# AhmedHumais/E-RAFT

Measured on AMD Instinct MI355X. Metric: CorrBlock build+lookup frame-pairs/sec & HBM GB/s at DSEC 480×640, 1–8 GPUs, higher is better.
Workload: dtype f32; 1 GPU; CorrBlock build + 12 lookups, dsec fmaps [1,256,60,80], 4 levels, radius 4; global_batch=1, launch=hipgraph, parallelism=replicas x1 (independent frame pairs per GPU)

## Files before the change

### e-raft_amd/csrc/corr_build_bf16.hip

```cpp
#include <algorithm>
#include <atomic>
#include <cmath>

#include "corr_build_common.h"

namespace corr {

typedef __bf16 bfx8_t __attribute__((ext_vector_type(8)));
typedef unsigned u32x4_t __attribute__((ext_vector_type(4)));
typedef float f32x4_t __attribute__((ext_vector_type(4)));

namespace bf16b {

constexpr int kStepK = 32;
constexpr int kPieces = 3;
constexpr int kRecU = kPieces * 64;
constexpr int kPatchRows = 8;
constexpr int kWaves = 4, kQPerWave = 32;
constexpr int kQPerWG = kWaves * kQPerWave;
constexpr int kRing = 3;
constexpr int kSlotBytes = kPatchRows * kPieces * 1024;
constexpr int kLds = kRing * kSlotBytes;
constexpr int kDmaPerWave = kPatchRows * kPieces / kWaves;
constexpr int kQLoads = 2 * kPieces;
constexpr int kPixBytes = kStepK * kPieces * 2;

struct Geom {
    int S, NQp, NQB, NQG, Hp, CB, Wp;
};

inline Geom geom(int D, int NQ, int H, int W) {
    Geom g;
    g.S = (D + kStepK - 1) / kStepK;
    g.NQp = (NQ + kQPerWG - 1) / kQPerWG * kQPerWG;
    g.NQB = g.NQp / 16;
    g.NQG = g.NQp / kQPerWG;
    g.Hp = (H + kPatchRows - 1) / kPatchRows * kPatchRows;
    g.CB = (W + 15) / 16;
    g.Wp = g.CB * 16;
    return g;
}

struct PackArgs {
    const float *f[2];
    u32x4_t *pk[2];
    int np[2];
    int nblk[2];
    int img[2];
    int D, S, W, CB, y0, y1, z0;
};

template <int R = 1>
__global__ __launch_bounds__(256) void bf16_pack_kernel(PackArgs a) {
    const int z = blockIdx.z + a.z0, b = blockIdx.y;
    const int nblk = a.nblk[z];
    const int lane = threadIdx.x & 63, ci = lane & 15, grp = lane >> 4;
    const int NP = a.np[z];
    float v[R][8];
    bool live[R];
    size_t dst[R];
#pragma unroll
    for (int r = 0; r < R; ++r) {
        const int rec = (blockIdx.x * R + r) * 4 + (threadIdx.x >> 6);
        live[r] = rec < a.S * nblk;
        const int s = live[r] ? rec / nblk : 0, blk = live[r] ? rec - s * nblk : 0;
        int n, iblk;
        bool valid;
        if (z == 0) {
            n = blk * 16 + ci;
            valid = n < a.np[0];
            iblk = blk;
        } else {
            const int TCp = 4 * a.CB, ty = blk / TCp, tx = blk - ty * TCp;
            const int ly = 4 * ty + (ci >> 2), x = 4 * tx + (ci & 3);
            valid = a.y0 + ly < a.y1 && x < a.W;
            n = ly * a.W + x;
            iblk = (a.y0 >> 2) * TCp + blk;
        }
        valid = valid && live[r];
        const int k0 = s * kStepK + 8 * grp;
        const float *src = a.f[z] + (size_t)b * a.D * NP + (valid ? n : 0);
#pragma unroll
        for (int j = 0; j < 8; ++j) v[r][j] = (valid && k0 + j < a.D) ? src[(size_t)(k0 + j) * NP] : 0.f;
        dst[r] = (((size_t)b * a.S + s) * a.img[z] + iblk) * kRecU + lane;
    }
#pragma unroll
    for (int r = 0; r < R; ++r) {
        if (!live[r]) continue;
        unsigned hh[4], mm[4], ll[4];
#pragma unroll
        for (int j = 0; j < 4; ++j) split3(v[r][2 * j], v[r][2 * j + 1], hh[j], mm[j], ll[j]);
        const u32x4_t h{hh[0], hh[1], hh[2], hh[3]}, m{mm[0], mm[1], mm[2], mm[3]}, l{ll[0], ll[1], ll[2], ll[3]};
        u32x4_t *out = a.pk[z] + dst[r];
        out[0] = h;
        out[64] = m;
        out[128] = l;
    }
}

struct Args {
    const u32x4_t *pq, *pt;
    float *lvl[kFusedLevels];
    int B, H, W, N, NQ, S, nlev;
    int NQp, NQB, NQG, Hp, CB, npatch;
    int py0;
    int exact;
    float inv_s, s;
    int order;
    int gq;
    int nqh, npq;
};

__device__ __forceinline__ Tile xcd_block_tile(const Args &p, int t) {
    Tile o;
    const int per_b = p.npatch * p.NQG;
    o.b = t / per_b;
    int r = t - o.b * per_b;
    int q0 = 0, q1 = 0, p0 = 0, p1 = 0;
    for (int i = 0; i < p.nqh; ++i) {
        const int qa = i * p.NQG / p.nqh, qb = (i + 1) * p.NQG / p.nqh;
        const int rows = (qb - qa) * p.npatch;
        if (r < rows) {
            for (int j = 0; j < p.npq; ++j) {
                const int pa = j * p.npatch / p.npq, pb = (j + 1) * p.npatch / p.npq;
                const int sz = (qb - qa) * (pb - pa);
                if (r < sz) {
                    q0 = qa, q1 = qb, p0 = pa, p1 = pb;
                    break;
                }
                r -= sz;
            }
            break;
        }
        r -= rows;
    }
    (void)q1;
    const int np = p1 - p0;
    o.qg = q0 + r / np;
    const int patch = p0 + r % np;
    o.py = patch / p.CB;
    o.cb = patch - o.py * p.CB;
    return o;
}

template <int SS, int NR, bool ACC2, int VF = 0, bool FAST = false>
__device__ __forceinline__ void build_tile(const Args &p, const Tile tl) {
    constexpr int QS = ACC2 ? 3 : 4, QD = QS - 1;
    constexpr int WV = kWaves, QPWG = kQPerWG, DPW = kDmaPerWave;
    extern __shared__ __attribute__((aligned(16))) char smem_bf16[];
    char *smem = smem_bf16;

    const int b = tl.b, y0 = tl.py * kPatchRows, x0 = tl.cb * 16;
    const int tid = threadIdx.x, lane = tid & 63;
    const int w = __builtin_amdgcn_readfirstlane(tid >> 6);
    const int ci = lane & 15, grp = lane >> 4;
    const int qb0 = tl.qg * (QPWG / 16) + 2 * w;
    const int S = SS > 0 ? SS : p.S;
    const bool qact = qb0 * 16 < p.NQ;

    const int TCp = 4 * p.CB;
    const size_t tstep = (size_t)p.Hp * p.CB * kRecU;
    const u32x4_t *tbase = p.pt + (((size_t)b * S * (p.Hp >> 2) + (y0 >> 2)) * TCp + 4 * tl.cb) * kRecU + lane;
    unsigned toff[DPW];
#pragma unroll
    for (int m = 0; m < DPW; ++m) {
        const int pc = w + WV * m, rp = pc / kPieces;
        toff[m] = (unsigned)(((rp >> 2) * TCp + (rp & 3)) * kRecU + (pc % kPieces) * 64);
    }
    const size_t qstep = (size_t)p.NQB * kRecU;
    const uint32_t lds_base = (uint32_t)(uintptr_t)(lds_void_t *)smem;
    const u32x4_t *qsrc = p.pq + ((size_t)b * S * p.NQB + qb0) * kRecU + lane;

    u32x4_t qv[QS][2][kPieces];
    auto issue_q = [&](int s, int slot) __attribute__((always_inline)) {
#pragma unroll
        for (int i = 0; i < 2; ++i)
#pragma unroll
            for (int c = 0; c < kPieces; ++c) {
                if constexpr (VF & 1)
                    asm volatile("global_load_dwordx4 %0, %1, off" : "=v"(qv[slot][i][c]) : "v"(qsrc + s * qstep + i * kRecU + c * 64) : "memory");
                else
                    qv[slot][i][c] = qsrc[s * qstep + i * kRecU + c * 64];
            }
    };
    auto issue_t = [&](int s, int slot) __attribute__((always_inline)) {
        const uint32_t base = lds_base + slot * kSlotBytes;
        const u32x4_t *src = tbase + s * tstep;
#pragma unroll
        for (int m = 0; m < DPW; ++m) dma16(src + toff[m], base + (w + WV * m) * 1024);
    };

    f32x4_t acc[2][kPatchRows], acs[2][kPatchRows];
#pragma unroll
    for (int i = 0; i < 2; ++i)
#pragma unroll
        for (int r = 0; r < kPatchRows; ++r) acc[i][r] = acs[i][r] = f32x4_t{0.f, 0.f, 0.f, 0.f};

    auto compute = [&](int tslot, int qslot) __attribute__((always_inline)) {
        const u32x4_t *A = reinterpret_cast<const u32x4_t *>(smem + tslot * kSlotBytes);
        bfx8_t qh[2], qm[2], ql[2];
#pragma unroll
        for (int i = 0; i < 2; ++i) {
            qh[i] = __builtin_bit_cast(bfx8_t, qv[qslot][i][0]);
            qm[i] = __builtin_bit_cast(bfx8_t, qv[qslot][i][1]);
            ql[i] = __builtin_bit_cast(bfx8_t, qv[qslot][i][2]);
        }
        bfx8_t th[2], tm[2], tl8[2];
        th[0] = __builtin_bit_cast(bfx8_t, A[lane]);
        tm[0] = __builtin_bit_cast(bfx8_t, A[64 + lane]);
        tl8[0] = __builtin_bit_cast(bfx8_t, A[128 + lane]);
        if constexpr (ACC2) {
#pragma unroll
            for (int r = 0; r < NR; ++r) {
                const int c = r & 1;
                if (r + 1 < NR) {
                    th[c ^ 1] = __builtin_bit_cast(bfx8_t, A[(3 * r + 3) * 64 + lane]);
                    tm[c ^ 1] = __builtin_bit_cast(bfx8_t, A[(3 * r + 4) * 64 + lane]);
                    tl8[c ^ 1] = __builtin_bit_cast(bfx8_t, A[(3 * r + 5) * 64 + lane]);
                }
#pragma unroll
                for (int i = 0; i < 2; ++i) acs[i][r] = __builtin_amdgcn_mfma_f32_16x16x32_bf16(tl8[c], qh[i], acs[i][r], 0, 0, 0);
#pragma unroll
                for (int i = 0; i < 2; ++i) acs[i][r] = __builtin_amdgcn_mfma_f32_16x16x32_bf16(th[c], ql[i], acs[i][r], 0, 0, 0);
#pragma unroll
                for (int i = 0; i < 2; ++i) acs[i][r] = __builtin_amdgcn_mfma_f32_16x16x32_bf16(tm[c], qm[i], acs[i][r], 0, 0, 0);
#pragma unroll
                for (int i = 0; i < 2; ++i) acs[i][r] = __builtin_amdgcn_mfma_f32_16x16x32_bf16(tm[c], qh[i], acs[i][r], 0, 0, 0);
#pragma unroll
                for (int i = 0; i < 2; ++i) acs[i][r] = __builtin_amdgcn_mfma_f32_16x16x32_bf16(th[c], qm[i], acs[i][r], 0, 0, 0);
#pragma unroll
                for (int i = 0; i < 2; ++i) acc[i][r] = __builtin_amdgcn_mfma_f32_16x16x32_bf16(th[c], qh[i], acc[i][r], 0, 0, 0);
            }
            __builtin_amdgcn_sched_group_barrier(0x100, 3, 0);
#pragma unroll
            for (int r = 0; r < NR; ++r) {
                if (r + 1 < NR) __builtin_amdgcn_sched_group_barrier(0x100, 3, 0);
                __builtin_amdgcn_sched_group_barrier(0x008, 12, 0);
            }
        } else {
            f32x4_t t[2][2];
#pragma unroll
            for (int r = 0; r < NR; ++r) {
                const int c = r & 1;
                if (r + 1 < NR) {
                    th[c ^ 1] = __builtin_bit_cast(bfx8_t, A[(3 * r + 3) * 64 + lane]);
                    tm[c ^ 1] = __builtin_bit_cast(bfx8_t, A[(3 * r + 4) * 64 + lane]);
                    tl8[c ^ 1] = __builtin_bit_cast(bfx8_t, A[(3 * r + 5) * 64 + lane]);
                }
                const f32x4_t z = {0.f, 0.f, 0.f, 0.f};
#pragma unroll
                for (int i = 0; i < 2; ++i) t[c][i] = __builtin_amdgcn_mfma_f32_16x16x32_bf16(tl8[c], qh[i], z, 0, 0, 0);
#pragma unroll
                for (int i = 0; i < 2; ++i) t[c][i] = __builtin_amdgcn_mfma_f32_16x16x32_bf16(th[c], ql[i], t[c][i], 0, 0, 0);
#pragma unroll
                for (int i = 0; i < 2; ++i) t[c][i] = __builtin_amdgcn_mfma_f32_16x16x32_bf16(tm[c], qm[i], t[c][i], 0, 0, 0);
#pragma unroll
                for (int i = 0; i < 2; ++i) t[c][i] = __builtin_amdgcn_mfma_f32_16x16x32_bf16(tm[c], qh[i], t[c][i], 0, 0, 0);
#pragma unroll
                for (int i = 0; i < 2; ++i) t[c][i] = __builtin_amdgcn_mfma_f32_16x16x32_bf16(th[c], qm[i], t[c][i], 0, 0, 0);
#pragma unroll
                for (int i = 0; i < 2; ++i) t[c][i] = __builtin_amdgcn_mfma_f32_16x16x32_bf16(th[c], qh[i], t[c][i], 0, 0, 0);
                if (r > 0) {
#pragma unroll
                    for (int i = 0; i < 2; ++i) acc[i][r - 1] += t[c ^ 1][i];
                }
            }
#pragma unroll
            for (int i = 0; i < 2; ++i) acc[i][NR - 1] += t[(NR - 1) & 1][i];
            __builtin_amdgcn_sched_group_barrier(0x100, 3, 0);
#pragma unroll
            for (int r = 0; r < NR; ++r) {
                if (r + 1 < NR) __builtin_amdgcn_sched_group_barrier(0x100, 3, 0);
                __builtin_amdgcn_sched_group_barrier(0x008, 12, 0);
                if (r > 0) __builtin_amdgcn_sched_group_barrier(0x002, 8, 0);
            }
            __builtin_amdgcn_sched_group_barrier(0x002, 8, 0);
        }
    };

    if constexpr (SS > 0) {
        if constexpr ((VF & 2) != 0) __builtin_amdgcn_s_setprio(1);
        issue_q(0, 0);
        if (SS > 1) issue_q(1, 1);
        issue_t(0, 0);
        if (QD > 2 && SS > 2) issue_q(2, 2);
        if (SS > 1) issue_t(1, 1);
#pragma unroll
        for (int s = 0; s < SS; ++s) {
            const int younger = s == 0 ? (QD > 2 && SS > 2 ? kQLoads : 0) + (SS > 1 ? DPW : 0)
                                       : (s - 1 + QD < SS ? kQLoads : 0) + (s + 1 < SS ? DPW : 0);
            if (younger == kQLoads + DPW) wait_vmcnt_barrier<kQLoads + DPW>();
            else if (younger == DPW) wait_vmcnt_barrier<DPW>();
            else if (younger == kQLoads) wait_vmcnt_barrier<kQLoads>();
            else wait_vmcnt_barrier<0>();
            const int qs = s % QS;
#pragma unroll
            for (int i = 0; i < 2; ++i)
                asm volatile("" : "+v"(qv[qs][i][0]), "+v"(qv[qs][i][1]), "+v"(qv[qs][i][2]));
            if (s + QD < SS) issue_q(s + QD, (s + QD) % QS);
            if (s + 2 < SS) issue_t(s + 2, (s + 2) % kRing);
            if (qact) compute(s % kRing, qs);
        }
        if constexpr ((VF & 2) != 0) __builtin_amdgcn_s_setprio(0);
    } else {
        asm volatile("s_waitcnt vmcnt(0)" ::: "memory");
        for (int s = 0; s < S; ++s) {
            issue_q(s, 0);
            issue_t(s, 0);
            wait_vmcnt_barrier<0>();
            if (qact) compute(0, 0);
            asm volatile("s_waitcnt lgkmcnt(0)\n\ts_barrier" ::: "memory");
        }
    }

    const int H = p.H, W = p.W, NQ = p.NQ, nlev = FAST ? 4 : p.nlev;
    const int H1 = H >> 1, W1 = W >> 1, H2 = H >> 2, W2 = W >> 2, H3 = H >> 3, W3 = W >> 3;
    const int TC0 = map_tcols(W), TC1 = map_tcols(W1), TC2 = map_tcols(W2), TC3 = map_tcols(W3);
    const int R0 = 4 * map_tiles(H), R1 = 4 * map_tiles(H1), R2 = 4 * map_tiles(H2), R3 = 4 * map_tiles(H3);
    const size_t M0 = map_floats(H, W), M1 = map_floats(H1, W1), M2 = map_floats(H2, W2), M3 = map_floats(H3, W3);
    const int h = grp >> 1, k = grp & 1;
    float l2s[2][2];
#pragma unroll
    for (int i = 0; i < 2; ++i) {
        const int q = (qb0 + i) * 16 + ci;
        const bool qok = q < NQ;
        const size_t qrow = (size_t)b * NQ + q;
        float v[kPatchRows][4];
#pragma unroll
        for (int r = 0; r < kPatchRows; ++r)
#pragma unroll
            for (int g = 0; g < 4; ++g) v[r][g] = (ACC2 ? split_sum(acc[i][r][g], acs[i][r][g]) : acc[i][r][g]) * p.inv_s;
        if (qok && nlev > 0) {
            float *m0 = p.lvl[0] + qrow * M0;
#pragma unroll
            for (int rp = 0; rp < kPatchRows; ++rp) {
                const int Y = y0 + 4 * (rp >> 2) + grp, T = (x0 >> 2) + (rp & 3);
                if (Y < R0 && 4 * T < W)
                    *reinterpret_cast<float4 *>(m0 + map_row4(Y, T, TC0)) = make_float4(v[rp][0], v[rp][1], v[rp][2], v[rp][3]);
            }
        }
        float l1[2][4];
#pragma unroll
        for (int tr = 0; tr < 2; ++tr) {
            float top[2][4], bot[2][4];
#pragma unroll
            for (int j = 0; j < 2; ++j)
#pragma unroll
                for (int c = 0; c < 4; ++c) {
                    const float mine = k ? v[4 * tr + 2 + j][c] : v[4 * tr + j][c];
                    const float give = k ? v[4 * tr + j][c] : v[4 * tr + 2 + j][c];
                    const float got = __shfl_xor(give, 16);
                    top[j][c] = k ? got : mine;
                    bot[j][c] = k ? mine : got;
                }
#pragma unroll
            for (int m = 0; m < 4; ++m) {
                const int j = m >> 1, c = 2 * (m & 1);
                l1[tr][m] = pool4(top[j][c], top[j][c + 1], bot[j][c], bot[j][c + 1]);
            }
            const int Y1 = (y0 >> 1) + 2 * tr + h, T1 = (x0 >> 3) + k;
            if (qok && nlev > 1 && Y1 < R1 && 4 * T1 < W1)
                *reinterpret_cast<float4 *>(p.lvl[1] + qrow * M1 + map_row4(Y1, T1, TC1)) =
                    make_float4(l1[tr][0], l1[tr][1], l1[tr][2], l1[tr][3]);
        }
        float top[4], bot[4];
#pragma unroll
        for (int m = 0; m < 4; ++m) {
            const float give = h ? l1[0][m] : l1[1][m];
            const float got = __shfl_xor(give, 32);
            top[m] = h ? got : l1[0][m];
            bot[m] = h ? l1[1][m] : got;
        }
#pragma unroll
        for (int j = 0; j < 2; ++j) l2s[i][j] = pool4(top[2 * j], top[2 * j + 1], bot[2 * j], bot[2 * j + 1]);
    }
    {
        const float g0 = __shfl_xor(k ? l2s[0][0] : l2s[1][0], 16), g1 = __shfl_xor(k ? l2s[0][1] : l2s[1][1], 16);
        const float o0 = k ? l2s[1][0] : l2s[0][0], o1 = k ? l2s[1][1] : l2s[0][1];
        const float4 o = k ? make_float4(g0, g1, o0, o1) : make_float4(o0, o1, g0, g1);
        const int q = (qb0 + k) * 16 + ci, Y2 = (y0 >> 2) + h;
        if (q < NQ && nlev > 2 && Y2 < R2 && (x0 >> 2) < W2)
            *reinterpret_cast<float4 *>(p.lvl[2] + ((size_t)b * NQ + q) * M2 + map_row4(Y2, x0 >> 4, TC2)) = o;
    }
    {
        const float g0 = __shfl_xor(h ? l2s[0][0] : l2s[1][0], 32), g1 = __shfl_xor(h ? l2s[0][1] : l2s[1][1], 32);
        const float l3 = h ? pool4(g0, g1, l2s[1][0], l2s[1][1]) : pool4(l2s[0][0], l2s[0][1], g0, g1);
        const int q = (qb0 + h) * 16 + ci;
        const int Y3 = y0 >> 3, X3 = (x0 >> 3) + k;
        if (q < NQ && nlev > 3 && Y3 < R3 && X3 < kTileW * TC3) p.lvl[3][((size_t)b * NQ + q) * M3 + map_cell(Y3, X3, TC3)] = l3;
    }
}

template <int SS, bool ACC2 = true, int VF = 0, bool FAST = false>
__global__ __launch_bounds__(256, 2) void corr_build_bf16_kernel(Args p) {
    const int t = xcd_swizzle(blockIdx.x, gridDim.x);
    Tile tl = p.order == 2 ? xcd_block_tile(p, t) : patch_tile(t, p.npatch, p.NQG, p.CB, p.order, p.gq);
    tl.py += p.py0;
    if (!(VF & 4) && SS > 0 && tl.py * kPatchRows + kPatchRows / 2 >= p.H)
        build_tile<SS, kPatchRows / 2, ACC2, VF, FAST>(p, tl);
    else
        build_tile<SS, kPatchRows, ACC2, VF, FAST>(p, tl);
}

struct Ws {
    u32x4_t *pq, *pt;
};

inline Ws workspace_of(void *ws, int B, const Geom &g) {
    char *w = (char *)ws;
    Ws r;
    r.pq = (u32x4_t *)w;
    w += align256((size_t)B * g.S * g.NQp * kPixBytes);
    r.pt = (u32x4_t *)w;
    return r;
}

template <int SS, bool ACC2 = true, int VF = 0>
hipError_t launch_kernel(dim3 grid, const Args &p, hipStream_t s) {
    const bool fast = p.nlev == 4;
    static std::atomic<unsigned long long> lds_done[2];
    const void *fn = fast ? (const void *)corr_build_bf16_kernel<SS, ACC2, VF, true>
                          : (const void *)corr_build_bf16_kernel<SS, ACC2, VF, false>;
    const hipError_t e = ensure_lds_limit(fn, kLds, lds_done[fast]);
    if (e != hipSuccess) return e;
    const dim3 blk(256);
    if (fast)
        hipLaunchKernelGGL((corr_build_bf16_kernel<SS, ACC2, VF, true>), grid, blk, kLds, s, p);
    else
        hipLaunchKernelGGL((corr_build_bf16_kernel<SS, ACC2, VF, false>), grid, blk, kLds, s, p);
    return hipGetLastError();
}


size_t workspace_bytes(int B, int D, int NQ, int H, int W) {
    const Geom g = geom(D, NQ, H, W);
    return align256((size_t)B * g.S * g.NQp * kPixBytes) + align256((size_t)B * g.S * g.Hp * g.Wp * kPixBytes);
}

hipError_t launch_pack(const float *f1, int NQ, const float *f2, int B, int D, int H, int W, void *ws,
                       hipStream_t s, int y0 = 0, int y1 = -1, bool pack_q = true, int rpw = 0) {
    if (y1 < 0) y1 = H;
    const Geom g = geom(D, NQ, H, W);
    const Ws w = workspace_of(ws, B, g);
    PackArgs a{};
    a.f[0] = f1, a.f[1] = f2;
    a.pk[0] = w.pq, a.pk[1] = w.pt;
    a.np[0] = NQ, a.np[1] = (y1 - y0) * W;
    const int nyp = (y1 + kPatchRows - 1) / kPatchRows * kPatchRows - y0;
    a.nblk[0] = g.NQB, a.nblk[1] = nyp * g.CB;
    a.img[0] = g.NQB, a.img[1] = g.Hp * g.CB;
    a.D = D, a.S = g.S, a.W = W, a.CB = g.CB, a.y0 = y0, a.y1 = y1;
    a.z0 = pack_q ? 0 : 1;
    const int recs = g.S * std::max(pack_q ? a.nblk[0] : 0, a.nblk[1]);
    if (rpw == 0) rpw = (long)recs * B * (pack_q ? 2 : 1) >= 8192 ? 4 : 1;
    const dim3 blk(256);
    if (rpw == 4)
        hipLaunchKernelGGL(bf16_pack_kernel<4>, dim3((unsigned)((recs + 15) / 16), B, pack_q ? 2 : 1), blk, 0, s, a);
    else if (rpw == 2)
        hipLaunchKernelGGL(bf16_pack_kernel<2>, dim3((unsigned)((recs + 7) / 8), B, pack_q ? 2 : 1), blk, 0, s, a);
    else
        hipLaunchKernelGGL(bf16_pack_kernel<1>, dim3((unsigned)((recs + 3) / 4), B, pack_q ? 2 : 1), blk, 0, s, a);
    return hipGetLastError();
}

hipError_t launch_mfma(int NQ, int B, int D, int H, int W, int levels, const LevelPtrs &pyr, void *ws,
                       hipStream_t s, int variant = 0, int order = 1, int y0 = 0, int y1 = -1, int gq = 0) {
    if (y1 < 0) y1 = H;
    const Geom g = geom(D, NQ, H, W);
    const Ws w = workspace_of(ws, B, g);
    Args p{};
    p.pq = w.pq, p.pt = w.pt;
    p.B = B, p.H = H, p.W = W, p.N = H * W, p.NQ = NQ, p.S = g.S;
    p.nlev = std::min(levels, kFusedLevels);
    for (int l = 0; l < kFusedLevels; ++l) p.lvl[l] = l < p.nlev ? pyr.p[l] : nullptr;
    p.NQp = g.NQp, p.NQB = g.NQB, p.NQG = g.NQG, p.Hp = g.Hp, p.CB = g.CB;
    p.py0 = y0 / kPatchRows;
    p.npatch = ((y1 + kPatchRows - 1) / kPatchRows - p.py0) * g.CB;
    p.s = std::sqrt((float)D);
    p.inv_s = 1.0f / p.s;
    p.exact = is_pow2(p.s);
    p.order = order;
    p.gq = gq > 0 ? gq : (B == 1 ? 4 : kGroupQ);
    const int per = B >= 8 ? 1 : 8 / B;
    p.nqh = per >= 2 && g.NQG >= 2 ? 2 : 1;
    p.npq = std::max(1, std::min(per / p.nqh, p.npatch));
    const long tiles = (long)B * p.npatch * p.NQG;
    if (tiles > 0x7fffffffL) return hipErrorInvalidValue;
    const dim3 grid((unsigned)tiles);
    hipError_t e;
    if (variant != 0) {
        if (g.S != 8) return hipErrorInvalidValue;
        switch (variant) {
            case 1: e = launch_kernel<8, false>(grid, p, s); break;
            case 2: e = launch_kernel<8, true, 1>(grid, p, s); break;
            case 3: e = launch_kernel<8, true, 2>(grid, p, s); break;
            case 4: e = launch_kernel<8, true, 3>(grid, p, s); break;
            case 5: e = launch_kernel<8, true, 4>(grid, p, s); break;
            default: return hipErrorInvalidValue;
        }
    } else switch (g.S <= 8 ? g.S : 0) {
#define CORR_BF16_CASE(c) \
    case c: e = launch_kernel<c>(grid, p, s); break;
        CORR_BF16_CASE(0) CORR_BF16_CASE(1) CORR_BF16_CASE(2) CORR_BF16_CASE(3) CORR_BF16_CASE(4)
        CORR_BF16_CASE(5) CORR_BF16_CASE(6) CORR_BF16_CASE(7) CORR_BF16_CASE(8)
#undef CORR_BF16_CASE
        default: return hipErrorInvalidValue;
    }
    if (e != hipSuccess) return e;
    if (levels > kFusedLevels) return launch_pool_levels(pyr, kFusedLevels, levels, (long)B * NQ, H, W, s);
    return hipSuccess;
}

}

size_t build_bf16_workspace(int B, int D, int NQ, int H, int W) {
    return bf16b::workspace_bytes(B, D, NQ, H, W);
}

hipError_t launch_build_bf16(const float *f1, int NQ, const float *f2, int B, int D, int H, int W, int levels,
                             const LevelPtrs &pyr, void *ws, hipStream_t s, int part) {
    if (part != 2) {
        const hipError_t e = bf16b::launch_pack(f1, NQ, f2, B, D, H, W, ws, s);
        if (e != hipSuccess || part == 1) return e;
    }
    return bf16b::launch_mfma(NQ, B, D, H, W, levels, pyr, ws, s);
}

hipError_t launch_build_bf16_region(const float *f1, int NQ, const float *f2_rows, int y0, int y1, int B, int D,
                                    int H, int W, int levels, const LevelPtrs &pyr, void *ws, bool pack_q,
                                    hipStream_t s) {
    const hipError_t e = bf16b::launch_pack(f1, NQ, f2_rows, B, D, H, W, ws, s, y0, y1, pack_q);
    if (e != hipSuccess) return e;
    return bf16b::launch_mfma(NQ, B, D, H, W, levels, pyr, ws, s, 0, 1, y0, y1);
}

}
```

Measured before the change: 6772 frame-pairs/s.

## Streamline bf16 corr build epilogue with permlane swaps, fast path, and interior stores

Rewrites the epilogue of the bf16 correlation build kernel. Cross-lane pyramid pooling now uses v_permlane16/32_swap instead of __shfl_xor with selects. The split-sum accumulator merge becomes a plain vector add unless a wave-wide ballot detects an infinity. A bounds-check-free interior path handles the pyramid stores. The default VF template variant is also switched to 2, which turns on the setprio scheduling variant for the library path. Together these aim to cut ALU, cross-lane and predication overhead in the store phase, at the cost of inline asm hazards, a slightly different numeric merge in the non-inf case, and larger code.

```diff
diff --git a/e-raft_amd/csrc/corr_build_bf16.hip b/e-raft_amd/csrc/corr_build_bf16.hip
--- a/e-raft_amd/csrc/corr_build_bf16.hip
+++ b/e-raft_amd/csrc/corr_build_bf16.hip
@@ -1,6 +1,7 @@
 #include <algorithm>
 #include <atomic>
 #include <cmath>
+#include <type_traits>
 
 #include "corr_build_common.h"
 
@@ -28,6 +29,19 @@
 struct Geom {
     int S, NQp, NQB, NQG, Hp, CB, Wp;
 };
+
+#define CORR_SWAP_FNS(N)                                                                                               \
+    __device__ __forceinline__ void swap##N(float &x, float &z) {                                                      \
+        asm volatile("s_nop 1\n\tv_permlane" #N "_swap_b32 %0, %1" : "+v"(x), "+v"(z));                                \
+    }                                                                                                                  \
+    __device__ __forceinline__ void swap##N##x4(float (&x)[4], float (&z)[4]) {                                        \
+        asm volatile("s_nop 1\n\tv_permlane" #N "_swap_b32 %0, %4\n\tv_permlane" #N "_swap_b32 %1, %5\n\t"             \
+            "v_permlane" #N "_swap_b32 %2, %6\n\tv_permlane" #N "_swap_b32 %3, %7"                                     \
+            : "+v"(x[0]), "+v"(x[1]), "+v"(x[2]), "+v"(x[3]), "+v"(z[0]), "+v"(z[1]), "+v"(z[2]), "+v"(z[3]));         \
+    }
+CORR_SWAP_FNS(16)
+CORR_SWAP_FNS(32)
+#undef CORR_SWAP_FNS
 
 inline Geom geom(int D, int NQ, int H, int W) {
     Geom g;
@@ -319,76 +333,111 @@
     const int R0 = 4 * map_tiles(H), R1 = 4 * map_tiles(H1), R2 = 4 * map_tiles(H2), R3 = 4 * map_tiles(H3);
     const size_t M0 = map_floats(H, W), M1 = map_floats(H1, W1), M2 = map_floats(H2, W2), M3 = map_floats(H3, W3);
     const int h = grp >> 1, k = grp & 1;
-    float l2s[2][2];
-#pragma unroll
-    for (int i = 0; i < 2; ++i) {
-        const int q = (qb0 + i) * 16 + ci;
-        const bool qok = q < NQ;
-        const size_t qrow = (size_t)b * NQ + q;
-        float v[kPatchRows][4];
-#pragma unroll
-        for (int r = 0; r < kPatchRows; ++r)
-#pragma unroll
-            for (int g = 0; g < 4; ++g) v[r][g] = (ACC2 ? split_sum(acc[i][r][g], acs[i][r][g]) : acc[i][r][g]) * p.inv_s;
-        if (qok && nlev > 0) {
-            float *m0 = p.lvl[0] + qrow * M0;
-#pragma unroll
-            for (int rp = 0; rp < kPatchRows; ++rp) {
-                const int Y = y0 + 4 * (rp >> 2) + grp, T = (x0 >> 2) + (rp & 3);
-                if (Y < R0 && 4 * T < W)
-                    *reinterpret_cast<float4 *>(m0 + map_row4(Y, T, TC0)) = make_float4(v[rp][0], v[rp][1], v[rp][2], v[rp][3]);
-            }
-        }
-        float l1[2][4];
-#pragma unroll
-        for (int tr = 0; tr < 2; ++tr) {
-            float top[2][4], bot[2][4];
-#pragma unroll
-            for (int j = 0; j < 2; ++j)
-#pragma unroll
-                for (int c = 0; c < 4; ++c) {
-                    const float mine = k ? v[4 * tr + 2 + j][c] : v[4 * tr + j][c];
-                    const float give = k ? v[4 * tr + j][c] : v[4 * tr + 2 + j][c];
-                    const float got = __shfl_xor(give, 16);
-                    top[j][c] = k ? got : mine;
-                    bot[j][c] = k ? mine : got;
+
+    if constexpr (ACC2) {
+        float big = 0.f;
+#pragma unroll
+        for (int i = 0; i < 2; ++i)
+#pragma unroll
+            for (int r = 0; r < NR; ++r)
+#pragma unroll
+                for (int g = 0; g < 4; ++g) big = __builtin_fmaxf(big, __builtin_fabsf(acc[i][r][g]));
+        if (__builtin_amdgcn_ballot_w64(__builtin_isinf(big)) != 0) {
+#pragma unroll
+            for (int i = 0; i < 2; ++i)
+#pragma unroll
+                for (int r = 0; r < NR; ++r)
+#pragma unroll
+                    for (int g = 0; g < 4; ++g) acc[i][r][g] = split_sum(acc[i][r][g], acs[i][r][g]) * p.inv_s;
+        } else {
+#pragma unroll
+            for (int i = 0; i < 2; ++i)
+#pragma unroll
+                for (int r = 0; r < NR; ++r) acc[i][r] = (acc[i][r] + acs[i][r]) * p.inv_s;
+        }
+    } else {
+#pragma unroll
+        for (int i = 0; i < 2; ++i)
+#pragma unroll
+            for (int r = 0; r < NR; ++r) acc[i][r] = acc[i][r] * p.inv_s;
+    }
+
+    const bool interior = (qb0 + 2) * 16 <= NQ && y0 + NR <= R0 && x0 + 12 < W &&
+                          (nlev < 2 || ((y0 >> 1) + 4 <= R1 && 4 * ((x0 >> 3) + 1) < W1)) &&
+                          (nlev < 3 || ((y0 >> 2) + 2 <= R2 && (x0 >> 2) < W2)) &&
+                          (nlev < 4 || ((y0 >> 3) < R3 && (x0 >> 3) + 1 < kTileW * TC3));
+
+    auto pool_store = [&](auto edge) __attribute__((always_inline)) {
+        constexpr bool EDGE = decltype(edge)::value;
+        float l2s[2][2];
+#pragma unroll
+        for (int i = 0; i < 2; ++i) {
+            const int q = (qb0 + i) * 16 + ci;
+            const bool qok = !EDGE || q < NQ;
+            const size_t qrow = (size_t)b * NQ + q;
+            if (nlev > 0) {
+                float *m0 = p.lvl[0] + qrow * M0 + map_row4(y0 + grp, x0 >> 2, TC0);
+#pragma unroll
+                for (int rp = 0; rp < NR; ++rp) {
+                    float *dst = m0 + ((rp >> 2) * TC0 + (rp & 3)) * (4 * kTileW);
+                    if (!EDGE || (qok && y0 + 4 * (rp >> 2) + grp < R0 && 4 * ((x0 >> 2) + (rp & 3)) < W))
+                        *reinterpret_cast<f32x4_t *>(dst) = acc[i][rp];
                 }
-#pragma unroll
-            for (int m = 0; m < 4; ++m) {
-                const int j = m >> 1, c = 2 * (m & 1);
-                l1[tr][m] = pool4(top[j][c], top[j][c + 1], bot[j][c], bot[j][c + 1]);
-            }
-            const int Y1 = (y0 >> 1) + 2 * tr + h, T1 = (x0 >> 3) + k;
-            if (qok && nlev > 1 && Y1 < R1 && 4 * T1 < W1)
-                *reinterpret_cast<float4 *>(p.lvl[1] + qrow * M1 + map_row4(Y1, T1, TC1)) =
-                    make_float4(l1[tr][0], l1[tr][1], l1[tr][2], l1[tr][3]);
-        }
-        float top[4], bot[4];
-#pragma unroll
-        for (int m = 0; m < 4; ++m) {
-            const float give = h ? l1[0][m] : l1[1][m];
-            const float got = __shfl_xor(give, 32);
-            top[m] = h ? got : l1[0][m];
-            bot[m] = h ? l1[1][m] : got;
-        }
-#pragma unroll
-        for (int j = 0; j < 2; ++j) l2s[i][j] = pool4(top[2 * j], top[2 * j + 1], bot[2 * j], bot[2 * j + 1]);
-    }
-    {
-        const float g0 = __shfl_xor(k ? l2s[0][0] : l2s[1][0], 16), g1 = __shfl_xor(k ? l2s[0][1] : l2s[1][1], 16);
-        const float o0 = k ? l2s[1][0] : l2s[0][0], o1 = k ? l2s[1][1] : l2s[0][1];
-        const float4 o = k ? make_float4(g0, g1, o0, o1) : make_float4(o0, o1, g0, g1);
-        const int q = (qb0 + k) * 16 + ci, Y2 = (y0 >> 2) + h;
-        if (q < NQ && nlev > 2 && Y2 < R2 && (x0 >> 2) < W2)
-            *reinterpret_cast<float4 *>(p.lvl[2] + ((size_t)b * NQ + q) * M2 + map_row4(Y2, x0 >> 4, TC2)) = o;
-    }
-    {
-        const float g0 = __shfl_xor(h ? l2s[0][0] : l2s[1][0], 32), g1 = __shfl_xor(h ? l2s[0][1] : l2s[1][1], 32);
-        const float l3 = h ? pool4(g0, g1, l2s[1][0], l2s[1][1]) : pool4(l2s[0][0], l2s[0][1], g0, g1);
-        const int q = (qb0 + h) * 16 + ci;
-        const int Y3 = y0 >> 3, X3 = (x0 >> 3) + k;
-        if (q < NQ && nlev > 3 && Y3 < R3 && X3 < kTileW * TC3) p.lvl[3][((size_t)b * NQ + q) * M3 + map_cell(Y3, X3, TC3)] = l3;
-    }
+            }
+            float l1[2][4];
+#pragma unroll
+            for (int tr = 0; tr < 2; ++tr) {
+                if (4 * tr < NR) {
+                    float top[2][4], bot[2][4];
+#pragma unroll
+                    for (int j = 0; j < 2; ++j) {
+#pragma unroll
+                        for (int c = 0; c < 4; ++c) top[j][c] = acc[i][4 * tr + j][c], bot[j][c] = acc[i][4 * tr + 2 + j][c];
+                        swap16x4(top[j], bot[j]);
+                    }
+#pragma unroll
+                    for (int m = 0; m < 4; ++m) {
+                        const int j = m >> 1, c = 2 * (m & 1);
+                        l1[tr][m] = pool4(top[j][c], top[j][c + 1], bot[j][c], bot[j][c + 1]);
+                    }
+                } else {
+#pragma unroll
+                    for (int m = 0; m < 4; ++m) l1[tr][m] = 0.f;
+                }
+            }
+            if (nlev > 1) {
+                float *m1 = p.lvl[1] + qrow * M1 + map_row4((y0 >> 1) + h, (x0 >> 3) + k, TC1);
+#pragma unroll
+                for (int tr = 0; tr < 2; ++tr)
+                    if (!EDGE || (qok && (y0 >> 1) + 2 * tr + h < R1 && 4 * ((x0 >> 3) + k) < W1))
+                        *reinterpret_cast<f32x4_t *>(m1 + 2 * tr * kTileW) = f32x4_t{l1[tr][0], l1[tr][1], l1[tr][2], l1[tr][3]};
+            }
+            swap32x4(l1[0], l1[1]);
+#pragma unroll
+            for (int j = 0; j < 2; ++j) l2s[i][j] = pool4(l1[0][2 * j], l1[0][2 * j + 1], l1[1][2 * j], l1[1][2 * j + 1]);
+        }
+        {
+            float a0 = l2s[0][0], a1 = l2s[0][1], c0 = l2s[1][0], c1 = l2s[1][1];
+            swap16(a0, c0);
+            swap16(a1, c1);
+            const int q = (qb0 + k) * 16 + ci, Y2 = (y0 >> 2) + h;
+            if (nlev > 2 && (!EDGE || (q < NQ && Y2 < R2 && (x0 >> 2) < W2)))
+                *reinterpret_cast<f32x4_t *>(p.lvl[2] + ((size_t)b * NQ + q) * M2 + map_row4(Y2, x0 >> 4, TC2)) =
+                    f32x4_t{a0, a1, c0, c1};
+        }
+        {
+            float a0 = l2s[0][0], a1 = l2s[0][1], c0 = l2s[1][0], c1 = l2s[1][1];
+            swap32(a0, c0);
+            swap32(a1, c1);
+            const float l3 = pool4(a0, a1, c0, c1);
+            const int q = (qb0 + h) * 16 + ci;
+            const int Y3 = y0 >> 3, X3 = (x0 >> 3) + k;
+            if (nlev > 3 && (!EDGE || (q < NQ && Y3 < R3 && X3 < kTileW * TC3)))
+                p.lvl[3][((size_t)b * NQ + q) * M3 + map_cell(Y3, X3, TC3)] = l3;
+        }
+    };
+    if (interior) pool_store(std::false_type{});
+    else pool_store(std::true_type{});
 }
 
 template <int SS, bool ACC2 = true, int VF = 0, bool FAST = false>
@@ -415,7 +464,9 @@
     return r;
 }
 
-template <int SS, bool ACC2 = true, int VF = 0>
+constexpr int kLibVF = 2;
+
+template <int SS, bool ACC2 = true, int VF = kLibVF>
 hipError_t launch_kernel(dim3 grid, const Args &p, hipStream_t s) {
     const bool fast = p.nlev == 4;
     static std::atomic<unsigned long long> lds_done[2];
@@ -491,11 +542,12 @@
     if (variant != 0) {
         if (g.S != 8) return hipErrorInvalidValue;
         switch (variant) {
-            case 1: e = launch_kernel<8, false>(grid, p, s); break;
+            case 1: e = launch_kernel<8, false, 0>(grid, p, s); break;
             case 2: e = launch_kernel<8, true, 1>(grid, p, s); break;
             case 3: e = launch_kernel<8, true, 2>(grid, p, s); break;
             case 4: e = launch_kernel<8, true, 3>(grid, p, s); break;
             case 5: e = launch_kernel<8, true, 4>(grid, p, s); break;
+            case 6: e = launch_kernel<8, true, 0>(grid, p, s); break;
             default: return hipErrorInvalidValue;
         }
     } else switch (g.S <= 8 ? g.S : 0) {
```

Result: faster. 7158 frame-pairs/s, median of 6 (+5.7%).
